# chernistry/sentio

Measured on NVIDIA H100. Metric: retrieval queries/sec @1M docs,1024-d,top_k=100, higher is better.
Workload: dtype f16 store / f32 scan / f64 exact re-score

## Files before the change

sentio_b200/csrc/dense_mma.cu:

```cuda
#include <cuda.h>

#include <math.h>

#include <algorithm>
#include <vector>

#include "dense_common.cuh"
#include "dense_mma.cuh"
#include "wgmma.cuh"

namespace {

constexpr int kTileRows = 128;
constexpr int kBK = 64;
constexpr uint32_t kATileBytes = kTileRows * kBK * 2;
constexpr int kConsumerWarps = 8;
constexpr int kMmaThreads = 32 * kConsumerWarps + 32;
constexpr int kQbnMax = 256;
constexpr int kSampleRows = 16;
constexpr int kSampleKeys = kTileRows / kSampleRows;
constexpr int kSelectThreads = 512;
constexpr int kSelStage = 8192;
constexpr int kSelTop = 2048;

__device__ __forceinline__ void tma_load_2d(uint32_t dst, const CUtensorMap* map, int c0, int c1, uint32_t bar,
                                            uint64_t policy) {
  asm volatile(
      "cp.async.bulk.tensor.2d.shared::cluster.global.mbarrier::complete_tx::bytes.L2::cache_hint [%0], [%1, {%2, %3}], "
      "[%4], %5;" ::"r"(dst),
      "l"(map), "r"(c0), "r"(c1), "r"(bar), "l"(policy)
      : "memory");
}
__device__ __forceinline__ void tma_prefetch_l2_2d(const CUtensorMap* map, int c0, int c1) {
  asm volatile("cp.async.bulk.prefetch.tensor.2d.L2.global [%0, {%1, %2}];" ::"l"(map), "r"(c0), "r"(c1) : "memory");
}

struct MmaScanParams {
  const float* inv_norm;
  const float* thr_init;
  unsigned long long* cand;
  int32_t* counts;
  int32_t* fallback;
  int64_t n;
  int32_t kb_count;
  int32_t num_tiles;
  int32_t tile_first, tile_step;
  int32_t capg;
  int32_t stages;
  int32_t prefetch;
  const uint32_t* mask;
  int32_t mask_qs;
  const float* hh;
  const float* rq;
};

template <int QBN, bool FILTER, bool EUCLID>
__global__ void __launch_bounds__(kMmaThreads, 1)
dense_scan_mma_kernel(const __grid_constant__ CUtensorMap tm_rows, const __grid_constant__ CUtensorMap tm_q,
                      const MmaScanParams p) {
  extern __shared__ uint8_t msm_raw[];
  const uint32_t raw = smem_u32(msm_raw);
  const uint32_t base = (raw + 1023u) & ~1023u;
  uint8_t* sm = msm_raw + (base - raw);
  constexpr uint32_t kQBoxBytes = QBN * kBK * 2;
  constexpr uint32_t kStageBytes = kATileBytes + kQBoxBytes;
  uint64_t* bars = reinterpret_cast<uint64_t*>(sm + (size_t)p.stages * kStageBytes);
  const uint32_t bar_full = smem_u32(bars), bar_empty = smem_u32(bars + p.stages);
  volatile float* thr = reinterpret_cast<volatile float*>(bars + 2 * p.stages);
  int* cnt = reinterpret_cast<int*>(const_cast<float*>(thr) + QBN);
  float* rq_s = reinterpret_cast<float*>(cnt + QBN);

  const int warp = threadIdx.x >> 5, lane = threadIdx.x & 31;
  const int grid = gridDim.x, cta = blockIdx.x;
  const int my_tiles = cta < p.num_tiles ? (p.num_tiles - 1 - cta) / grid + 1 : 0;
  auto tile_row = [&](int t) { return (p.tile_first + (cta + t * grid) * p.tile_step) * kTileRows; };

  if (threadIdx.x == 0) {
    for (int s = 0; s < p.stages; ++s) {
      mbar_init(bar_full + 8 * s, 1);
      mbar_init(bar_empty + 8 * s, kConsumerWarps);
    }
    mbar_fence_init();
    asm volatile("prefetch.tensormap [%0];" ::"l"(&tm_rows) : "memory");
    asm volatile("prefetch.tensormap [%0];" ::"l"(&tm_q) : "memory");
  }
  for (int i = threadIdx.x; i < QBN; i += blockDim.x) {
    thr[i] = p.thr_init ? p.thr_init[i] : -INFINITY;
    cnt[i] = 0;
    if constexpr (EUCLID) rq_s[i] = p.rq[i];
  }
  __syncthreads();

  if (warp == kConsumerWarps) {
    if (lane == 0) {
      const uint64_t pol_corpus = policy_evict_first();
      const uint64_t pol_query = policy_evict_last();
      int it = 0;
      const int total_it = my_tiles * p.kb_count;
      for (int t = 0; t < my_tiles; ++t) {
        const int row = tile_row(t);
        for (int kb = 0; kb < p.kb_count; ++kb, ++it) {
          const int s = it % p.stages;
          const uint32_t use = (uint32_t)(it / p.stages);
          const int pf = it + p.stages + p.prefetch;
          if (p.prefetch > 0 && pf < total_it) {
            const int pt = pf / p.kb_count, pkb = pf - pt * p.kb_count;
            tma_prefetch_l2_2d(&tm_rows, pkb * kBK, tile_row(pt));
          }
          if (it >= p.stages) mbar_wait(bar_empty + 8 * s, (use & 1u) ^ 1u);
          const uint32_t stage = base + (uint32_t)s * kStageBytes;
          mbar_expect_tx(bar_full + 8 * s, kStageBytes);
          tma_load_2d(stage, &tm_rows, kb * kBK, row, bar_full + 8 * s, pol_corpus);
          tma_load_2d(stage + kATileBytes, &tm_q, kb * kBK, 0, bar_full + 8 * s, pol_query);
        }
      }
    }
  } else {
    const int wg = warp >> 2;
    unsigned long long* my_cand = p.cand + (size_t)cta * p.capg;
    const size_t q_stride = (size_t)grid * p.capg;
    int it = 0;
    for (int t = 0; t < my_tiles; ++t) {
      float acc[QBN / 2];
      for (int kb = 0; kb < p.kb_count; ++kb, ++it) {
        const int s = it % p.stages;
        mbar_wait(bar_full + 8 * s, (uint32_t)(it / p.stages) & 1u);
        const uint32_t stage = base + (uint32_t)s * kStageBytes;
        const uint64_t da = wgmma_desc_sw128(stage + (uint32_t)wg * (kATileBytes / 2));
        const uint64_t db = wgmma_desc_sw128(stage + kATileBytes);
        wgmma_fence();
#pragma unroll
        for (int k = 0; k < kBK / 16; ++k)
          Wgmma<QBN>::mma(acc, da + (uint64_t)(2 * k), db + (uint64_t)(2 * k), (kb | k) ? 1u : 0u);
        wgmma_commit();
        wgmma_wait<1>();
        __syncwarp();
        if (kb > 0 && lane == 0) mbar_arrive(bar_empty + 8 * ((it - 1) % p.stages));
      }
      wgmma_wait<0>();
      __syncwarp();
      if (lane == 0) mbar_arrive(bar_empty + 8 * ((it - 1) % p.stages));
      const int64_t row0 = (int64_t)tile_row(t) + wg * 64 + (warp & 3) * 16 + (lane >> 2);
      const bool live0 = row0 < p.n, live1 = row0 + 8 < p.n;
      const float invn0 = live0 ? __ldg(p.inv_norm + row0) : 0.f;
      const float invn1 = live1 ? __ldg(p.inv_norm + row0 + 8) : 0.f;
      float h0 = 0.f, h1 = 0.f;
      if constexpr (EUCLID) {
        h0 = live0 ? __ldg(p.hh + row0) : 0.f;
        h1 = live1 ? __ldg(p.hh + row0 + 8) : 0.f;
      }
      auto key = [&](float a, float invn, float h, int col) {
        float s = a * invn;
        if constexpr (EUCLID) s = __fsub_rn(__fmul_rn(rq_s[col], s), h);
        return s;
      };
      const uint32_t* mrow = nullptr;
      if constexpr (FILTER) mrow = p.mask + (size_t)(row0 >> 5) * p.mask_qs + 2 * (lane & 3);
      const int sh0 = (int)(row0 & 31), sh1 = sh0 + 8;
      if (p.thr_init == nullptr) {
        const int slot = t * kSampleKeys + warp;
#pragma unroll
        for (int j = 0; j < QBN / 4; j += 2) {
          uint2 mw = make_uint2(0u, 0u);
          if constexpr (FILTER) mw = __ldg(reinterpret_cast<const uint2*>(mrow + 4 * j));
#pragma unroll
          for (int e = 0; e < 2; ++e) {
            bool m0 = live0, m1 = live1;
            if constexpr (FILTER) {
              const uint32_t w = e ? mw.y : mw.x;
              m0 = m0 && ((w >> sh0) & 1u);
              m1 = m1 && ((w >> sh1) & 1u);
            }
            const int col = 4 * j + 2 * (lane & 3) + e;
            const float s0 = m0 ? key(acc[2 * j + e], invn0, h0, col) : -INFINITY;
            const float s1 = m1 ? key(acc[2 * j + 2 + e], invn1, h1, col) : -INFINITY;
            uint32_t best = max(f32_orderable(s0), f32_orderable(s1));
            best = max(best, __shfl_xor_sync(0xffffffffu, best, 4));
            best = max(best, __shfl_xor_sync(0xffffffffu, best, 8));
            best = max(best, __shfl_xor_sync(0xffffffffu, best, 16));
            if (lane < 4) my_cand[(size_t)col * q_stride + slot] = ((unsigned long long)best << 32) | 0xffffffffull;
          }
        }
      } else {
#pragma unroll
        for (int j = 0; j < QBN / 4; j += 2) {
          uint2 mw = make_uint2(0u, 0u);
          if constexpr (FILTER) mw = __ldg(reinterpret_cast<const uint2*>(mrow + 4 * j));
#pragma unroll
          for (int h = 0; h < 2; ++h) {
            if (!(h ? live1 : live0)) continue;
            const int64_t row = row0 + 8 * h;
            const float invn = h ? invn1 : invn0;
            const float hrow = h ? h1 : h0;
#pragma unroll
            for (int e = 0; e < 2; ++e) {
              const int col = 4 * j + 2 * (lane & 3) + e;
              const float score = key(acc[2 * j + 2 * h + e], invn, hrow, col);
              bool match = true;
              if constexpr (FILTER) match = ((e ? mw.y : mw.x) >> (h ? sh1 : sh0)) & 1u;
              if (score >= thr[col] && match) {
                const int pos = atomicAdd(&cnt[col], 1);
                if (pos < p.capg) my_cand[(size_t)col * q_stride + pos] = make_key32(score, (uint32_t)row);
              }
            }
          }
        }
      }
    }
  }
  __syncthreads();
  for (int i = threadIdx.x; i < QBN; i += blockDim.x) {
    const int c = p.thr_init == nullptr ? my_tiles * kSampleKeys : cnt[i];
    p.counts[(size_t)i * grid + cta] = min(c, p.capg);
    if (c > p.capg && p.fallback) p.fallback[i] = 1;
  }
}

struct SelectParams {
  const unsigned long long* cand;
  const int32_t* counts;
  int32_t grid, capg;
  int32_t nq;
  int32_t mode;
  float* thr_out;
  const float* eps;
  int32_t* fallback;
  const __half* rows;
  const float* q;
  int32_t d_pad, ch;
  int64_t id_base;
  int32_t k;
  int64_t* out_ids;
  double* out_scores;
  int32_t* out_counts;
  const int32_t* state;
  int32_t metric;
  const double* cfac;
};

template <bool FILTER>
__global__ void __launch_bounds__(kSelectThreads, 2) dense_select_kernel(const SelectParams p) {
  extern __shared__ __align__(16) uint8_t ssm[];
  unsigned long long* keys = reinterpret_cast<unsigned long long*>(ssm);
  unsigned long long* top = keys + kSelStage;
  unsigned long long* ek = top + kSelTop;
  uint32_t* ei = reinterpret_cast<uint32_t*>(ek + kSelTop);
  __shared__ double qq_s;
  __shared__ int s_prefix[kSelectThreads + 1];
  __shared__ int s_hist[256];
  __shared__ int s_scal[4];
  __shared__ int s_ntop;
  const int tid = threadIdx.x, nt = blockDim.x, lane = tid & 31, warp = tid >> 5, nw = nt >> 5, qi = blockIdx.x;
  const int K = p.k, G = p.grid;
  if (p.mode == 0 && qi >= p.nq) {
    if (tid == 0) p.thr_out[qi] = INFINITY;
    return;
  }
  if constexpr (FILTER) {
    if (p.state[qi]) {
      if (p.mode == 0 && tid == 0) p.thr_out[qi] = INFINITY;
      return;
    }
  }
  if (p.fallback[qi] != 0) {
    if (p.mode == 0 && tid == 0) p.thr_out[qi] = INFINITY;
    return;
  }
  const int32_t* counts = p.counts + (size_t)qi * G;
  const unsigned long long* cand = p.cand + (size_t)qi * G * p.capg;
  {
    const int v = tid < G ? counts[tid] : 0;
    int x = v;
    for (int o = 1; o < 32; o <<= 1) {
      const int y = __shfl_up_sync(0xffffffffu, x, o);
      if (lane >= o) x += y;
    }
    if (lane == 31) s_hist[warp] = x;
    if (tid == 0) s_ntop = 0;
    __syncthreads();
    if (warp == 0) {
      int w = lane < nw ? s_hist[lane] : 0;
      for (int o = 1; o < 32; o <<= 1) {
        const int y = __shfl_up_sync(0xffffffffu, w, o);
        if (lane >= o) w += y;
      }
      s_hist[32 + lane] = w;
    }
    __syncthreads();
    const int incl = x + (warp ? s_hist[32 + warp - 1] : 0);
    if (tid < G) s_prefix[tid] = incl - v;
    if (tid == G - 1) s_prefix[G] = incl;
    __syncthreads();
  }
  const int total = s_prefix[G];
  const bool staged = total <= kSelStage;
  if (staged) {
    for (int g = warp; g < G; g += nw) {
      const int c = s_prefix[g + 1] - s_prefix[g];
      const unsigned long long* src = cand + (size_t)g * p.capg;
      unsigned long long* dst = keys + s_prefix[g];
      for (int i = lane; i < c; i += 32) dst[i] = src[i];
    }
    __syncthreads();
  }
#define SB_FOR_EACH_KEY(BODY)                                                       \
  if (staged) {                                                                     \
    for (int i_ = tid; i_ < total; i_ += nt) {                                      \
      const unsigned long long key = keys[i_];                                      \
      BODY                                                                          \
    }                                                                               \
  } else {                                                                          \
    for (int g_ = warp; g_ < G; g_ += nw) {                                         \
      const int c_ = s_prefix[g_ + 1] - s_prefix[g_];                               \
      const unsigned long long* src_ = cand + (size_t)g_ * p.capg;                  \
      for (int i_ = lane; i_ < c_; i_ += 32) {                                      \
        const unsigned long long key = src_[i_];                                    \
        BODY                                                                        \
      }                                                                             \
    }                                                                               \
  }

  unsigned long long prefix = 0ull, mask = 0ull;
  if (total > K) {
    int need = K;
    for (int shift = 56; shift >= 0; shift -= 8) {
      for (int i = tid; i < 256; i += nt) s_hist[i] = 0;
      __syncthreads();
      SB_FOR_EACH_KEY(if ((key & mask) == prefix) {
        const int dgt = (int)((key >> shift) & 0xffull);
        const unsigned grp = __match_any_sync(__activemask(), dgt);
        if ((int)(threadIdx.x & 31) == __ffs(grp) - 1) atomicAdd(&s_hist[dgt], __popc(grp));
      })
      __syncthreads();
      if (warp == 0) warp_select_bin<true>(s_hist, need, lane, s_scal);
      __syncthreads();
      prefix |= (unsigned long long)s_scal[0] << shift;
      mask |= 0xffull << shift;
      need = s_scal[1];
      const int bucket = s_scal[2];
      __syncthreads();
      if (bucket <= 16) break;
    }
  }
  const float eps = p.eps[qi];
  const unsigned long long lo_key = total > K ? window_lo_key(prefix, eps) : 0ull;
  if (p.mode == 0) {
    if (tid == 0) p.thr_out[qi] = total > K ? key32_score(lo_key) : -INFINITY;
    return;
  }
  SB_FOR_EACH_KEY(if (key >= lo_key) {
    const int at = atomicAdd(&s_ntop, 1);
    if (at < kSelTop) top[at] = key;
  })
#undef SB_FOR_EACH_KEY
  __syncthreads();
  const int ntop = s_ntop;
  if (ntop > kSelTop) {
    if (tid == 0) p.fallback[qi] = 1;
    return;
  }
  int P = 32;
  while (P < ntop) P <<= 1;
  RescoreArgs ra;
  ra.rows = p.rows;
  ra.q = p.q + (size_t)qi * p.d_pad;
  ra.d_pad = p.d_pad;
  ra.ch = p.ch;
  ra.id_base = p.id_base;
  ra.k = p.k;
  ra.out_ids = p.out_ids + (size_t)qi * p.k;
  ra.out_scores = p.out_scores + (size_t)qi * p.k;
  ra.out_count = p.out_counts + qi;
  ra.metric = p.metric;
  ra.cfac = p.cfac;
  rescore_and_emit(top, ntop, P, ek, ei, &qq_s, reinterpret_cast<float*>(keys), ra);
}

typedef CUresult (*EncodeTiledFn)(CUtensorMap*, CUtensorMapDataType, cuuint32_t, void*, const cuuint64_t*,
                                  const cuuint64_t*, const cuuint32_t*, const cuuint32_t*, CUtensorMapInterleave,
                                  CUtensorMapSwizzle, CUtensorMapL2promotion, CUtensorMapFloatOOBfill);

int encode_map(CUtensorMap* map, const void* ptr, int64_t rows, int64_t cols, int box_rows) {
  static EncodeTiledFn fn = nullptr;
  if (!fn) {
    void* pfn = nullptr;
    cudaDriverEntryPointQueryResult qres;
    if (cudaGetDriverEntryPoint("cuTensorMapEncodeTiled", &pfn, cudaEnableDefault, &qres) == cudaSuccess &&
        qres == cudaDriverEntryPointSuccess)
      fn = reinterpret_cast<EncodeTiledFn>(pfn);
  }
  SB_REQUIRE(fn != nullptr, SB_ERR_CUDA, "cuTensorMapEncodeTiled entry point not available");
  cuuint64_t dims[2] = {(cuuint64_t)cols, (cuuint64_t)rows};
  cuuint64_t strides[1] = {(cuuint64_t)cols * 2};
  cuuint32_t box[2] = {(cuuint32_t)kBK, (cuuint32_t)box_rows};
  cuuint32_t estr[2] = {1, 1};
  CUresult r = fn(map, CU_TENSOR_MAP_DATA_TYPE_FLOAT16, 2, const_cast<void*>(ptr), dims, strides, box, estr,
                  CU_TENSOR_MAP_INTERLEAVE_NONE, CU_TENSOR_MAP_SWIZZLE_128B, CU_TENSOR_MAP_L2_PROMOTION_L2_256B,
                  CU_TENSOR_MAP_FLOAT_OOB_FILL_NONE);
  SB_REQUIRE(r == CUDA_SUCCESS, SB_ERR_CUDA, "cuTensorMapEncodeTiled failed with CUresult %d", (int)r);
  return SB_OK;
}

size_t mma_per_query(bool euclid) { return euclid ? 12 : 8; }
int mma_stages(const sb_ctx* ctx, int qbn, bool euclid = false) {
  const size_t stage = kATileBytes + (size_t)qbn * kBK * 2 + 16;
  const size_t fixed = 1024 + (size_t)qbn * mma_per_query(euclid);
  return std::min((int)((ctx->smem_optin - fixed) / stage), ctx->dense_max_stages);
}
size_t mma_smem(int qbn, int stages, bool euclid) {
  return 1024 + (size_t)stages * (kATileBytes + (size_t)qbn * kBK * 2 + 16) + (size_t)qbn * mma_per_query(euclid);
}

template <int QBN, bool FILTER, bool EUCLID>
int launch_mma(const CUtensorMap& tm_rows, const CUtensorMap& tm_q, const MmaScanParams& mp, int grid, size_t smem,
               cudaStream_t st) {
  auto kern = dense_scan_mma_kernel<QBN, FILTER, EUCLID>;
  SB_CUDA(cudaFuncSetAttribute(kern, cudaFuncAttributeMaxDynamicSharedMemorySize, (int)smem));
  kern<<<grid, kMmaThreads, smem, st>>>(tm_rows, tm_q, mp);
  SB_CUDA(cudaGetLastError());
  return SB_OK;
}

template <bool FILTER, bool EUCLID>
int dispatch_mma(int qbn, const CUtensorMap& tm_rows, const CUtensorMap& tm_q, const MmaScanParams& mp, int grid,
                 size_t smem, cudaStream_t st) {
  switch (qbn) {
    case 16: return launch_mma<16, FILTER, EUCLID>(tm_rows, tm_q, mp, grid, smem, st);
    case 32: return launch_mma<32, FILTER, EUCLID>(tm_rows, tm_q, mp, grid, smem, st);
    case 64: return launch_mma<64, FILTER, EUCLID>(tm_rows, tm_q, mp, grid, smem, st);
    case 128: return launch_mma<128, FILTER, EUCLID>(tm_rows, tm_q, mp, grid, smem, st);
    case 256: return launch_mma<256, FILTER, EUCLID>(tm_rows, tm_q, mp, grid, smem, st);
  }
  sb_set_error("dense_mma: unsupported query block %d", qbn);
  return SB_ERR_UNSUPPORTED;
}

}

bool dense_mma_eligible(const sb_ctx* ctx, const DenseIndex& ix, int B) {
  if (B < 16) return false;
  if (ix.d_pad % kBK != 0 || ix.n_pad % kTileRows != 0) return false;
  if (ix.n < 64 * kTileRows) return false;
  return mma_stages(ctx, kQbnMax) >= 3;
}

int dense_mma_topk_enqueue(sb_ctx* ctx, DenseIndex& ix, const float* q_pad, int B, int k, int64_t* out_ids,
                           double* out_scores, int32_t* out_counts, cudaStream_t st, const DenseFilter* flt) {
  const int kb_count = ix.d_pad / kBK;
  const int total_tiles = (int)(ix.n_pad / kTileRows);
  const int gsz = kQbnMax;
  const int grid = std::min(ctx->num_sms, total_tiles);
  const double phi = flt ? std::min(1.0, (double)std::max<int64_t>(flt->c_min, 1) / (double)ix.n) : 1.0;
  const double hit = flt ? 1.0 - pow(1.0 - phi, (double)kSampleRows) : 1.0;
  const double m_eff = flt ? (double)kSampleRows * phi / hit : (double)kSampleRows;
  const int per_cta = flt ? std::max(ctx->dense_sample_per_cta,
                                     (int)ceil(4.0 * k / ((double)kSampleKeys * hit * grid)))
                          : std::max(ctx->dense_sample_per_cta, std::min(8, (4 * k / kSampleKeys + grid - 1) / grid));
  const int sample_tiles = (int)std::min<int64_t>((int64_t)per_cta * grid, total_tiles);
  const int sample_step = total_tiles / sample_tiles;
  const int sgrid = std::min(grid, sample_tiles);
  const int64_t worst = (int64_t)((total_tiles + grid - 1) / grid + 1) * kTileRows;
  const int64_t samp_keys = (int64_t)((sample_tiles + sgrid - 1) / sgrid + 1) * kSampleKeys;
  const double f = (double)k / ((double)kSampleKeys * sample_tiles * hit);
  const double pass = f >= 0.95 ? 1.0 : -log(1.0 - f) / m_eff;
  const int64_t expect = (int64_t)((double)worst * phi * pass) + 1;
  const int capg = (int)std::min<int64_t>(worst, std::max<int64_t>(8 * expect + 256, samp_keys));
  int rc;
  SB_REQUIRE(grid <= kSelectThreads, SB_ERR_UNSUPPORTED, "dense_mma: %d CTAs exceed the select kernel's prefix width", grid);
  const int n_groups = (B + gsz - 1) / gsz;
  const size_t cand_per_group = (size_t)gsz * grid * capg * 8;
  int gmax = (int)std::max<size_t>(1, (size_t)(1024ull << 20) / cand_per_group);
  gmax = std::min(gmax, n_groups);
  if ((rc = ctx->misc2_dev.reserve((size_t)n_groups * gsz * ix.d_pad * 2 + 256))) return rc;
  if ((rc = ctx->misc3_dev.reserve(((size_t)gsz * 4 + (size_t)gsz * grid * 4) * gmax + 256))) return rc;
  if ((rc = ctx->cand_dev.reserve(cand_per_group * gmax))) return rc;
  __half* q16 = ctx->misc2_dev.as<__half>();
  float* thr = ctx->misc3_dev.as<float>();
  int32_t* counts = reinterpret_cast<int32_t*>(thr + (size_t)gsz * gmax);
  unsigned long long* cand = ctx->cand_dev.as<unsigned long long>();
  if (ix.tm_rows_ptr != ix.rows || ix.tm_n_pad != ix.n_pad) {
    if ((rc = encode_map(reinterpret_cast<CUtensorMap*>(ix.tm_rows), ix.rows, ix.n_pad, ix.d_pad, kTileRows))) return rc;
    ix.tm_rows_ptr = ix.rows;
    ix.tm_n_pad = ix.n_pad;
  }
  const CUtensorMap& tm_rows = *reinterpret_cast<const CUtensorMap*>(ix.tm_rows);
  const size_t sel_smem = (size_t)kSelStage * 8 + (size_t)kSelTop * 20 + 64;
  if (flt) SB_CUDA(cudaFuncSetAttribute(dense_select_kernel<true>, cudaFuncAttributeMaxDynamicSharedMemorySize,
                                        (int)sel_smem));
  else SB_CUDA(cudaFuncSetAttribute(dense_select_kernel<false>, cudaFuncAttributeMaxDynamicSharedMemorySize,
                                    (int)sel_smem));
  auto launch_select = [&](int nblocks, const SelectParams& s) {
    if (flt) dense_select_kernel<true><<<nblocks, kSelectThreads, sel_smem, st>>>(s);
    else dense_select_kernel<false><<<nblocks, kSelectThreads, sel_smem, st>>>(s);
  };
  const bool euclid = ix.metric == SB_METRIC_EUCLID;
  auto run_mma = [&](int qbn, const CUtensorMap& tm_q, const MmaScanParams& m, int g, size_t smem) {
    if (euclid)
      return flt ? dispatch_mma<true, true>(qbn, tm_rows, tm_q, m, g, smem, st)
                 : dispatch_mma<false, true>(qbn, tm_rows, tm_q, m, g, smem, st);
    return flt ? dispatch_mma<true, false>(qbn, tm_rows, tm_q, m, g, smem, st)
               : dispatch_mma<false, false>(qbn, tm_rows, tm_q, m, g, smem, st);
  };
  float *eps = nullptr, *rq = nullptr;
  int32_t* fb = nullptr;
  if ((rc = dense_prep_queries(ctx, ix, q_pad, B, n_groups * gsz, true, nullptr, q16, &eps, &fb, &rq, st)))
    return rc;

  for (int c0 = 0; c0 < B; c0 += gmax * gsz) {
    const int nq_chunk = std::min(B - c0, gmax * gsz);
    const int ng = (nq_chunk + gsz - 1) / gsz;
    struct Group { int qbn, nq; CUtensorMap tm_q; size_t smem; int stages; };
    std::vector<Group> gs((size_t)ng);
    int rows_total = 0;
    for (int g = 0; g < ng; ++g) {
      Group& G = gs[(size_t)g];
      const int left = nq_chunk - g * gsz;
      __half* q16g = q16 + (size_t)(c0 + g * gsz) * ix.d_pad;
      G.qbn = gsz;
      while (G.qbn > 16 && G.qbn / 2 >= left) G.qbn >>= 1;
      G.nq = std::min(G.qbn, left);
      if ((rc = encode_map(&G.tm_q, q16g, G.qbn, ix.d_pad, G.qbn))) return rc;
      G.stages = mma_stages(ctx, G.qbn, euclid);
      G.smem = mma_smem(G.qbn, G.stages, euclid);
      rows_total = g * gsz + G.qbn;
    }
    MmaScanParams mp;
    mp.inv_norm = ix.inv_norm;
    mp.n = ix.n;
    mp.kb_count = kb_count;
    mp.capg = capg;
    mp.prefetch = ctx->dense_prefetch;
    mp.mask_qs = flt ? flt->qs : 0;
    mp.hh = ix.hh;
    SelectParams sp;
    sp.metric = ix.metric;
    sp.cfac = ix.cfac;
    sp.cand = cand;
    sp.counts = counts;
    sp.capg = capg;
    sp.nq = nq_chunk;
    sp.thr_out = thr;
    sp.eps = eps + c0;
    sp.fallback = fb + c0;
    sp.rows = ix.rows;
    sp.q = q_pad + (size_t)c0 * ix.d_pad;
    sp.d_pad = ix.d_pad;
    sp.ch = ix.d_pad / 8;
    sp.id_base = ix.id_base;
    sp.k = k;
    sp.out_ids = out_ids + (size_t)c0 * k;
    sp.out_scores = out_scores + (size_t)c0 * k;
    sp.out_counts = out_counts + c0;
    sp.state = flt ? flt->state + c0 : nullptr;
    mp.thr_init = nullptr;
    mp.fallback = nullptr;
    mp.num_tiles = sample_tiles;
    mp.tile_first = 0;
    mp.tile_step = sample_step;
    {
      ProfScope ps(ctx, SB_PROF_DENSE_SAMPLE, st, ng + 1);
      for (int g = 0; g < ng; ++g) {
        const Group& G = gs[(size_t)g];
        mp.cand = cand + (size_t)g * gsz * sgrid * capg;
        mp.counts = counts + (size_t)g * gsz * sgrid;
        mp.stages = G.stages;
        mp.mask = flt ? flt->mask + c0 + (size_t)g * gsz : nullptr;
        mp.rq = rq ? rq + c0 + (size_t)g * gsz : nullptr;
        if ((rc = run_mma(G.qbn, G.tm_q, mp, sgrid, G.smem))) return rc;
      }
      sp.grid = sgrid;
      sp.mode = 0;
      launch_select(rows_total, sp);
    }
    SB_CUDA(cudaGetLastError());
    mp.num_tiles = total_tiles;
    mp.tile_first = 0;
    mp.tile_step = 1;
    for (int g = 0; g < ng; ++g) {
      const Group& G = gs[(size_t)g];
      mp.thr_init = thr + (size_t)g * gsz;
      mp.fallback = fb + c0 + (size_t)g * gsz;
      mp.cand = cand + (size_t)g * gsz * grid * capg;
      mp.counts = counts + (size_t)g * gsz * grid;
      mp.stages = G.stages;
      mp.mask = flt ? flt->mask + c0 + (size_t)g * gsz : nullptr;
      mp.rq = rq ? rq + c0 + (size_t)g * gsz : nullptr;
      ProfScope ps(ctx, SB_PROF_DENSE_SCAN, st);
      if ((rc = run_mma(G.qbn, G.tm_q, mp, grid, G.smem))) return rc;
    }
    sp.grid = grid;
    sp.mode = 1;
    {
      ProfScope ps(ctx, SB_PROF_DENSE_MERGE, st);
      launch_select(nq_chunk, sp);
    }
    SB_CUDA(cudaGetLastError());
  }
  return dense_fallback_enqueue(ctx, ix, q_pad, B, k, fb, out_ids, out_scores, out_counts, st, flt);
}
```

Measured before the change: 141,500.

## Drop dedicated producer warp, use 3 consumer warpgroups with inline TMA refill

Grows the corpus tile from 128 to 192 rows so three consumer warpgroups each run wgmma on 64 rows, and removes the dedicated TMA producer warp. Thread 0 now issues the initial loads and refills each stage itself after waiting on the empty barrier. The epilogue threshold test first builds a pass bitmask from a vectorized read of the non-volatile threshold array, then does atomics only for passing entries. Having thread 0 block on the empty barrier may stall its warp's compute, and the larger tile raises smem per stage, which can reduce the stage count. Probe macros are added but off by default.

```diff
diff --git a/sentio_b200/csrc/dense_mma.cu b/sentio_b200/csrc/dense_mma.cu
--- a/sentio_b200/csrc/dense_mma.cu
+++ b/sentio_b200/csrc/dense_mma.cu
@@ -11,11 +11,13 @@
 
 namespace {
 
-constexpr int kTileRows = 128;
+constexpr int kTileRows = 192;
 constexpr int kBK = 64;
+constexpr uint32_t kWgRowsBytes = 64 * kBK * 2;
 constexpr uint32_t kATileBytes = kTileRows * kBK * 2;
-constexpr int kConsumerWarps = 8;
-constexpr int kMmaThreads = 32 * kConsumerWarps + 32;
+constexpr int kConsumerWarps = kTileRows / 16;
+constexpr int kMmaThreads = 32 * kConsumerWarps;
+constexpr int64_t kMmaMinRows = 8192;
 constexpr int kQbnMax = 256;
 constexpr int kSampleRows = 16;
 constexpr int kSampleKeys = kTileRows / kSampleRows;
@@ -66,8 +68,8 @@
   constexpr uint32_t kStageBytes = kATileBytes + kQBoxBytes;
   uint64_t* bars = reinterpret_cast<uint64_t*>(sm + (size_t)p.stages * kStageBytes);
   const uint32_t bar_full = smem_u32(bars), bar_empty = smem_u32(bars + p.stages);
-  volatile float* thr = reinterpret_cast<volatile float*>(bars + 2 * p.stages);
-  int* cnt = reinterpret_cast<int*>(const_cast<float*>(thr) + QBN);
+  float* thr = reinterpret_cast<float*>(bars + 2 * p.stages);
+  int* cnt = reinterpret_cast<int*>(thr + QBN);
   float* rq_s = reinterpret_cast<float*>(cnt + QBN);
 
   const int warp = threadIdx.x >> 5, lane = threadIdx.x & 31;
@@ -91,31 +93,38 @@
   }
   __syncthreads();
 
-  if (warp == kConsumerWarps) {
-    if (lane == 0) {
-      const uint64_t pol_corpus = policy_evict_first();
-      const uint64_t pol_query = policy_evict_last();
-      int it = 0;
-      const int total_it = my_tiles * p.kb_count;
-      for (int t = 0; t < my_tiles; ++t) {
-        const int row = tile_row(t);
-        for (int kb = 0; kb < p.kb_count; ++kb, ++it) {
-          const int s = it % p.stages;
-          const uint32_t use = (uint32_t)(it / p.stages);
-          const int pf = it + p.stages + p.prefetch;
-          if (p.prefetch > 0 && pf < total_it) {
-            const int pt = pf / p.kb_count, pkb = pf - pt * p.kb_count;
-            tma_prefetch_l2_2d(&tm_rows, pkb * kBK, tile_row(pt));
-          }
-          if (it >= p.stages) mbar_wait(bar_empty + 8 * s, (use & 1u) ^ 1u);
-          const uint32_t stage = base + (uint32_t)s * kStageBytes;
-          mbar_expect_tx(bar_full + 8 * s, kStageBytes);
-          tma_load_2d(stage, &tm_rows, kb * kBK, row, bar_full + 8 * s, pol_corpus);
-          tma_load_2d(stage + kATileBytes, &tm_q, kb * kBK, 0, bar_full + 8 * s, pol_query);
-        }
-      }
-    }
-  } else {
+  const int total_it = my_tiles * p.kb_count;
+  auto load = [&](int i) {
+    const int s = i % p.stages;
+    const int t = i / p.kb_count, kb = i - t * p.kb_count;
+    const int pf = i + p.stages + p.prefetch;
+    if (p.prefetch > 0 && pf < total_it) {
+      const int pt = pf / p.kb_count, pkb = pf - pt * p.kb_count;
+      tma_prefetch_l2_2d(&tm_rows, pkb * kBK, tile_row(pt));
+    }
+    const uint32_t stage = base + (uint32_t)s * kStageBytes;
+#ifdef SB_PROBE_QUERY_ONCE
+    const bool load_q = i < p.stages;
+#else
+    const bool load_q = true;
+#endif
+    mbar_expect_tx(bar_full + 8 * s, load_q ? kStageBytes : kATileBytes);
+    tma_load_2d(stage, &tm_rows, kb * kBK, tile_row(t), bar_full + 8 * s, policy_evict_first());
+    if (load_q) tma_load_2d(stage + kATileBytes, &tm_q, kb * kBK, 0, bar_full + 8 * s, policy_evict_last());
+  };
+  if (threadIdx.x == 0)
+    for (int i = 0; i < min(p.stages, total_it); ++i) load(i);
+  auto release = [&](int r) {
+    __syncwarp();
+    const int s = r % p.stages;
+    if (lane == 0) mbar_arrive(bar_empty + 8 * s);
+    if (threadIdx.x == 0 && r + p.stages < total_it) {
+      mbar_wait(bar_empty + 8 * s, (uint32_t)(r / p.stages) & 1u);
+      load(r + p.stages);
+    }
+    __syncwarp();
+  };
+  {
     const int wg = warp >> 2;
     unsigned long long* my_cand = p.cand + (size_t)cta * p.capg;
     const size_t q_stride = (size_t)grid * p.capg;
@@ -126,7 +135,7 @@
         const int s = it % p.stages;
         mbar_wait(bar_full + 8 * s, (uint32_t)(it / p.stages) & 1u);
         const uint32_t stage = base + (uint32_t)s * kStageBytes;
-        const uint64_t da = wgmma_desc_sw128(stage + (uint32_t)wg * (kATileBytes / 2));
+        const uint64_t da = wgmma_desc_sw128(stage + (uint32_t)wg * kWgRowsBytes);
         const uint64_t db = wgmma_desc_sw128(stage + kATileBytes);
         wgmma_fence();
 #pragma unroll
@@ -134,12 +143,19 @@
           Wgmma<QBN>::mma(acc, da + (uint64_t)(2 * k), db + (uint64_t)(2 * k), (kb | k) ? 1u : 0u);
         wgmma_commit();
         wgmma_wait<1>();
-        __syncwarp();
-        if (kb > 0 && lane == 0) mbar_arrive(bar_empty + 8 * ((it - 1) % p.stages));
+        if (kb > 0) release(it - 1);
       }
       wgmma_wait<0>();
-      __syncwarp();
-      if (lane == 0) mbar_arrive(bar_empty + 8 * ((it - 1) % p.stages));
+      release(it - 1);
+#ifdef SB_PROBE_NO_EPILOGUE
+      if (p.thr_init != nullptr) {
+        float sink = 0.f;
+#pragma unroll
+        for (int i = 0; i < QBN / 2; ++i) sink += acc[i];
+        if (sink == 1.2345e-30f) cnt[0] = 1;
+        continue;
+      }
+#endif
       const int64_t row0 = (int64_t)tile_row(t) + wg * 64 + (warp & 3) * 16 + (lane >> 2);
       const bool live0 = row0 < p.n, live1 = row0 + 8 < p.n;
       const float invn0 = live0 ? __ldg(p.inv_norm + row0) : 0.f;
@@ -162,7 +178,7 @@
 #pragma unroll
         for (int j = 0; j < QBN / 4; j += 2) {
           uint2 mw = make_uint2(0u, 0u);
-          if constexpr (FILTER) mw = __ldg(reinterpret_cast<const uint2*>(mrow + 4 * j));
+          if constexpr (FILTER) if (live0) mw = __ldg(reinterpret_cast<const uint2*>(mrow + 4 * j));
 #pragma unroll
           for (int e = 0; e < 2; ++e) {
             bool m0 = live0, m1 = live1;
@@ -185,23 +201,25 @@
 #pragma unroll
         for (int j = 0; j < QBN / 4; j += 2) {
           uint2 mw = make_uint2(0u, 0u);
-          if constexpr (FILTER) mw = __ldg(reinterpret_cast<const uint2*>(mrow + 4 * j));
+          if constexpr (FILTER) if (live0) mw = __ldg(reinterpret_cast<const uint2*>(mrow + 4 * j));
+          const float2 t2 = *reinterpret_cast<const float2*>(thr + 4 * j + 2 * (lane & 3));
+          uint32_t pass = 0u;
 #pragma unroll
-          for (int h = 0; h < 2; ++h) {
-            if (!(h ? live1 : live0)) continue;
-            const int64_t row = row0 + 8 * h;
-            const float invn = h ? invn1 : invn0;
-            const float hrow = h ? h1 : h0;
+          for (int u = 0; u < 4; ++u) {
+            const int h = u >> 1, e = u & 1;
+            const float score = key(acc[2 * j + u], h ? invn1 : invn0, h ? h1 : h0, 4 * j + 2 * (lane & 3) + e);
+            bool ok = (h ? live1 : live0) && score >= (e ? t2.y : t2.x);
+            if constexpr (FILTER) ok = ok && (((e ? mw.y : mw.x) >> (h ? sh1 : sh0)) & 1u);
+            pass |= (uint32_t)ok << u;
+          }
+          if (pass) {
 #pragma unroll
-            for (int e = 0; e < 2; ++e) {
-              const int col = 4 * j + 2 * (lane & 3) + e;
-              const float score = key(acc[2 * j + 2 * h + e], invn, hrow, col);
-              bool match = true;
-              if constexpr (FILTER) match = ((e ? mw.y : mw.x) >> (h ? sh1 : sh0)) & 1u;
-              if (score >= thr[col] && match) {
-                const int pos = atomicAdd(&cnt[col], 1);
-                if (pos < p.capg) my_cand[(size_t)col * q_stride + pos] = make_key32(score, (uint32_t)row);
-              }
+            for (int u = 0; u < 4; ++u) {
+              if (!((pass >> u) & 1u)) continue;
+              const int h = u >> 1, col = 4 * j + 2 * (lane & 3) + (u & 1);
+              const float score = key(acc[2 * j + u], h ? invn1 : invn0, h ? h1 : h0, col);
+              const int pos = atomicAdd(&cnt[col], 1);
+              if (pos < p.capg) my_cand[(size_t)col * q_stride + pos] = make_key32(score, (uint32_t)(row0 + 8 * h));
             }
           }
         }
@@ -439,15 +457,15 @@
 
 bool dense_mma_eligible(const sb_ctx* ctx, const DenseIndex& ix, int B) {
   if (B < 16) return false;
-  if (ix.d_pad % kBK != 0 || ix.n_pad % kTileRows != 0) return false;
-  if (ix.n < 64 * kTileRows) return false;
+  if (ix.d_pad % kBK != 0) return false;
+  if (ix.n < kMmaMinRows) return false;
   return mma_stages(ctx, kQbnMax) >= 3;
 }
 
 int dense_mma_topk_enqueue(sb_ctx* ctx, DenseIndex& ix, const float* q_pad, int B, int k, int64_t* out_ids,
                            double* out_scores, int32_t* out_counts, cudaStream_t st, const DenseFilter* flt) {
   const int kb_count = ix.d_pad / kBK;
-  const int total_tiles = (int)(ix.n_pad / kTileRows);
+  const int total_tiles = (int)((ix.n_pad + kTileRows - 1) / kTileRows);
   const int gsz = kQbnMax;
   const int grid = std::min(ctx->num_sms, total_tiles);
   const double phi = flt ? std::min(1.0, (double)std::max<int64_t>(flt->c_min, 1) / (double)ix.n) : 1.0;
```

Measured after the change: 149,100 (median of 6 runs). +5.3%, better.
